# mpkuse/cerebro

Measured on AMD Instinct MI355X. Metric: loop-queries/sec (ticks of 3 descriptors vs 4096-D x 1M DB), higher is better.
Workload: dtype f64

## Files before the change

cerebro_amd/csrc/chip_api.hip:

```cpp
#include "chip_internal.h"
#include <cmath>
#include <cstdlib>
#include <cstring>
#include <memory>
#include <new>

using namespace chip;

extern "C" {

const char *chip_strerror(int status)
{
    switch (status) {
        case CHIP_OK: return "ok";
        case CHIP_ERR_INVALID_ARG: return "invalid argument";
        case CHIP_ERR_NO_DEVICE: return "no usable HIP device";
        case CHIP_ERR_HIP: return "HIP runtime error (see chip_last_hip_error)";
        case CHIP_ERR_OOM: return "out of device memory";
        case CHIP_ERR_NOT_F32: return "descriptor value not exactly representable as float32";
        case CHIP_ERR_NONFINITE: return "NaN/Inf in descriptor";
        case CHIP_ERR_RANGE: return "index / length out of range";
        case CHIP_ERR_UNSUPPORTED: return "unsupported configuration";
        case CHIP_ERR_TOO_FEW_POINTS: return "fewer than 20 correspondences";
        case CHIP_ERR_BUSY: return "async slot busy or empty";
// ... 157 lines not shown
    c->scan_overlap_bytes = (double)env_int("CHIP_SCAN_OVERLAP_GIB", 8) * 1024 * 1024 * 1024;
    c->scan_reserve = env_int("CHIP_SCAN_RESERVE", c->nranks > 1 ? 4 : 0);
    c->max_grid = 512;
    c->scan_streams = env_int("CHIP_SCAN_STREAMS", c->nranks > 1 ? 2 : 4);
    c->tick_fused = env_int("CHIP_TICK_FUSED", 1) != 0;
}

static int create_impl(chip_ctx *c, int64_t capacity_hint, int elem)
{
    hipDeviceProp_t prop;
    CHIP_HIP(c, hipGetDeviceProperties(&prop, c->device));
    c->n_cus = prop.multiProcessorCount;
    std::strncpy(c->arch, prop.gcnArchName, sizeof(c->arch) - 1);
    if (std::strncmp(c->arch, "gfx950", 6) != 0 && !std::getenv("CHIP_ALLOW_ANY_ARCH")) return CHIP_ERR_NO_DEVICE;

    c->segs.reserve(kMaxSegs);

    CHIP_HIP(c, hipStreamCreateWithFlags(&c->s_query, hipStreamNonBlocking));
    CHIP_HIP(c, hipStreamCreateWithFlags(&c->s_append, hipStreamNonBlocking));
    CHIP_HIP(c, hipStreamCreateWithFlags(&c->s_pnp, hipStreamNonBlocking));
    int rc = c->seg_table_dev.alloc(c, kMaxSegs);
    if (rc == CHIP_OK) rc = configure_storage(c, elem);
    if (rc != CHIP_OK) return rc;
    c->stage_bytes = 64ull << 20;
    if (c->stage_bytes < (size_t)c->D * 8 * 64) c->stage_bytes = (size_t)c->D * 8 * 64;
    rc = c->stage_dev.alloc(c, c->stage_bytes);
    if (rc == CHIP_OK) rc = c->flags_dev.alloc(c, 1);
    if (rc == CHIP_OK) rc = c->flags_host.alloc(c, 1);
    if (rc == CHIP_OK) rc = c->norm2_dev.alloc(c, 1);
    if (rc == CHIP_OK) rc = c->norm2_host.alloc(c, 1);
    if (rc != CHIP_OK) return rc;
    CHIP_HIP(c, hipMemset(c->norm2_dev, 0, sizeof(unsigned long long)));
    *c->norm2_host.host() = 0;

    scan_read_knobs(c);
    CHIP_HIP(c, hipStreamCreateWithFlags(&c->s_scan, hipStreamNonBlocking));
    {
        const int ns = c->scan_streams;
        if (ns >= 2) CHIP_HIP(c, hipStreamCreateWithFlags(&c->s_scan2, hipStreamNonBlocking));
        for (int i = 0; i < 2; i++)
            if (ns >= 3 + i) CHIP_HIP(c, hipStreamCreateWithFlags(&c->s_scan_x[i], hipStreamNonBlocking));
    }
    for (int i = 0; i < Ctx::kRing; i++) {
        constexpr size_t kListsPerGroup = 3 * kPrefilterTicks > CHIP_MAX_NQ ? 3 * kPrefilterTicks : CHIP_MAX_NQ;
        static_assert(kPrefilterTicks >= kMultiMaxTicks, "the list buffers are sized for the deepest pass");
        rc = c->partial_dev[i].alloc(c, ((size_t)c->max_grid + 1) * kListsPerGroup * CHIP_MAX_TOPK);
        if (rc != CHIP_OK) return rc;
        CHIP_HIP(c, hipEventCreateWithFlags(&c->ev_scan[i], hipEventDisableTiming));
        CHIP_HIP(c, hipEventCreateWithFlags(&c->ev_merged[i], hipEventDisableTiming));
    }
    rc = c->tickets_dev.alloc(c, Ctx::kRing);
    if (rc != CHIP_OK) return rc;
    CHIP_HIP(c, hipMemset(c->tickets_dev, 0, Ctx::kRing * sizeof(int32_t)));
    c->coalesce_max = env_int("CHIP_TICK_COALESCE", kPrefilterTicks);
    if (c->coalesce_max < 2) c->coalesce_max = 0;
    if (c->coalesce_max > kPrefilterTicks) c->coalesce_max = kPrefilterTicks;
    c->tick_poll = env_int("CHIP_TICK_POLL", 1) != 0;
    resident_read_knobs(c);
    rc = c->seq_all.alloc(c, CHIP_MAX_INFLIGHT);
    if (rc != CHIP_OK) return rc;
    std::memset(c->seq_all.host(), 0, sizeof(unsigned long long) * CHIP_MAX_INFLIGHT);
    rc = c->cert_all.alloc(c, CHIP_MAX_INFLIGHT * 4);
    if (rc != CHIP_OK) return rc;
    std::memset(c->cert_all.host(), 0, sizeof(uint32_t) * CHIP_MAX_INFLIGHT * 4);
    rc = c->topk.alloc(c, (size_t)CHIP_MAX_NQ * CHIP_MAX_TOPK);
    if (rc != CHIP_OK) return rc;
    for (Slot &s : c->slots) {
        CHIP_HIP(c, hipEventCreateWithFlags(&s.done, hipEventDisableTiming));
        rc = s.rec.alloc(c, 1);
        if (rc != CHIP_OK) return rc;
        s.seq_host = c->seq_all.host() + (&s - c->slots);
        s.seq_dev = c->seq_all.dev() + (&s - c->slots);
        s.cert_host = c->cert_all.host() + 4 * (&s - c->slots);
        s.cert_dev = c->cert_all.dev() + 4 * (&s - c->slots);
    }
    if (env_int("CHIP_SCAN_STAMPS", 0)) {
        rc = c->stamps_dev.alloc(c, (size_t)c->max_grid * 16 * 4 + 64);
        if (rc != CHIP_OK) return rc;
        CHIP_HIP(c, hipMemset(c->stamps_dev, 0, ((size_t)c->max_grid * 16 * 4 + 64) * sizeof(unsigned long long)));
    }
    rc = pnp_create(c);
    if (rc != CHIP_OK) return rc;
    c->cap_hint = capacity_hint;
    if (capacity_hint > 0) {
        std::lock_guard<std::mutex> lk(c->append_mu);
        rc = ensure_capacity(c, local_count(c, capacity_hint));
        if (rc != CHIP_OK) return rc;
    }
    return CHIP_OK;
}

int ctx_create(chip_ctx **out, int32_t D, int64_t capacity_hint, int32_t device, int32_t shard_rank, int32_t shard_count, uint32_t flags)
{
    if (!out) return CHIP_ERR_INVALID_ARG;
    *out = nullptr;
    if (D <= 0 || shard_count < 1 || shard_rank < 0 || shard_rank >= shard_count || capacity_hint < 0) return CHIP_ERR_INVALID_ARG;
    const uint32_t store = flags & kCreateStoreMask;
    if (store == kCreateStoreMask) return CHIP_ERR_INVALID_ARG;
    if (D % 4 != 0 || (size_t)D * 4 * CHIP_MAX_NQ > 160 * 1024) return CHIP_ERR_UNSUPPORTED;
    if (store == CHIP_CREATE_STORE_F64 && (size_t)D * 8 * 2 > 160 * 1024) return CHIP_ERR_UNSUPPORTED;
    int ndev = 0;
    if (hipGetDeviceCount(&ndev) != hipSuccess || ndev <= 0) return CHIP_ERR_NO_DEVICE;
    if (device < 0 || device >= ndev) return CHIP_ERR_NO_DEVICE;
    if (hipSetDevice(device) != hipSuccess) return CHIP_ERR_NO_DEVICE;
    chip_ctx *c = new (std::nothrow) chip_ctx();
    if (!c) return CHIP_ERR_OOM;
// ... 220 lines not shown
    const int rc = enqueue_scan_merge(c, rq, &done);
    if (rc != CHIP_OK) return rc;
    if (done.done_ev) s.wait_ev = done.done_ev;
    else { CHIP_HIP(c, hipEventRecord(s.done, done.merge_stream)); s.wait_ev = s.done; }
    s.pass_no = c->pass_no;
    s.state = c->tick_poll && done.fused ? SlotState::Poll : SlotState::Event;
    return CHIP_OK;
}

int coalesce_decide(int n_parked, int t_max, bool scan_running)
{
    if (t_max < 2) return kCoalesceLaunch;
    if (!scan_running) return n_parked > 0 ? kCoalesceParkFlush : kCoalesceLaunch;
    return n_parked + 1 >= t_max ? kCoalesceParkFlush : kCoalescePark;
}

static int coalesce_ticks_max(const Ctx *c, int64_t k, bool sync_tick)
{
    if (c->coalesce_max < 2 || sync_tick || c->nranks != 1 || c->xchg || c->parent || c->group || !c->own_query_stream) return 0;
    if ((double)k * c->D * c->elem <= c->scan_overlap_bytes) return 0;
    int fit = scan_multi_max_ticks(c);
    if (c->coalesce_max >= kPrefilterTicks && scan_prefilter_usable(c)) fit = kPrefilterTicks;
    const int t = fit < c->coalesce_max ? fit : c->coalesce_max;
    return t >= 2 ? t : 0;
}

static int coalesce_submit(Ctx *c, int T)
{
    const int b = (int)(c->n_enqueued++ % Ctx::kRing);
    const int K = CHIP_DEFAULT_TOPK;
    const bool prefilter = T == kPrefilterTicks;
    static_assert(kPrefilterTicks > kMultiMaxTicks, "a pass of kPrefilterTicks ticks is the prefilter's");
    PassArgs a{};
    scan_args_db(c, &a);
    a.K = K;
    a.partial = c->partial_dev[b];
    for (int t = 0; t < T; t++) {
        a.k[t] = c->parked[t].k;
        if (a.k[t] > a.n_rows) a.n_rows = a.k[t];
        for (int i = 0; i < 3; i++) a.q[3 * t + i] = c->parked[t].q[i];
    }
    const int grid = scan_multi_grid(c);
    double E = 0.0;
    if (prefilter) {
        std::lock_guard<std::mutex> lk(c->mu);
        E = prefilter_error_bound(c->D, c->row_norm_max);
    }
    if (hipEventQuery(c->ev_merged[b]) != hipSuccess) CHIP_HIP(c, hipStreamWaitEvent(c->s_scan, c->ev_merged[b], 0));
    hipEvent_t e1 = nullptr;
    int rc = c->prof_on ? prof_begin(c, c->s_scan, (double)a.n_rows * c->D * c->elem, &e1) : CHIP_OK;
    if (rc == CHIP_OK) rc = prefilter ? launch_scan_prefilter(c, c->s_scan, a, grid) : launch_scan_multi(c, c->s_scan, a, T, grid);
    if (rc != CHIP_OK) return rc;
    if (e1) CHIP_HIP(c, hipEventRecord(e1, c->s_scan));
    CHIP_HIP(c, hipEventRecord(c->ev_scan[b], c->s_scan));
    c->pass_ev = c->ev_scan[b];
    c->pass_no++;
    CHIP_HIP(c, hipStreamWaitEvent(c->s_query, c->ev_scan[b], 0));
    chip_topk_entry *exact = c->partial_dev[b] + (size_t)kPrefilterTicks * grid * 3 * K;
    if (prefilter) {
        RescoreArgs ra{};
        ra.seg_table = a.seg_table; ra.seg_shift = a.seg_shift; ra.seg_mask = a.seg_mask; ra.D = a.D; ra.K = K;
        ra.in = c->partial_dev[b]; ra.n_lists = grid; ra.wpb = 8;
        ra.E = E;
        ra.out = exact;
        for (int t = 0; t < T; t++) {
            const Ctx::ParkedTick &pt = c->parked[t];
            Slot &s = *pt.slot;
            ra.k[t] = pt.k;
            for (int i = 0; i < 3; i++) { ra.q[3 * t + i] = s.pf_q[i] = pt.q[i]; s.cert_host[i] = 0; }
            ra.cert[t] = s.cert_dev;
            s.prefilter = true; s.pf_k = pt.k; s.pf_p = pt.p;
        }
        rc = launch_rescore(c, c->s_query, ra);
        if (rc != CHIP_OK) return rc;
    }
    for (int t = 0; t < T; t++) {
        const Ctx::ParkedTick &pt = c->parked[t];
        if (prefilter) rc = launch_merge(c, c->s_query, merge_args(exact + (size_t)t * 3 * K, 1, K, nullptr, pt.slot->rec.dev(), pt.l, &pt.p), 3);
        else rc = launch_merge(c, c->s_query, merge_args(c->partial_dev[b] + (size_t)t * grid * 3 * K, grid, K, nullptr, pt.slot->rec.dev(), pt.l, &pt.p), 3);
        if (rc != CHIP_OK) return rc;
        CHIP_HIP(c, hipEventRecord(pt.slot->done, c->s_query));
        pt.slot->wait_ev = pt.slot->done;
        pt.slot->state = SlotState::Event;
        pt.slot->pass_no = c->pass_no;
    }
    CHIP_HIP(c, hipEventRecord(c->ev_merged[b], c->s_query));
    c->coalesce_passes++;
    c->coalesce_ticks += T;
    if (prefilter) { c->prefilter_passes++; c->prefilter_ticks += T; }
    return CHIP_OK;
}

int coalesce_flush(Ctx *c)
{
    const int T = c->n_parked;
    if (T == 0) return CHIP_OK;
    c->n_parked = 0;
    const Ctx::ParkedTick &p0 = c->parked[0];
    int rc;
    if (T == kPrefilterTicks && !scan_prefilter_usable(c)) {
        const Ctx::ParkedTick &pl = c->parked[T - 1];
        rc = coalesce_submit(c, T - 1);
        if (rc == CHIP_OK) rc = tick_submit(c, pl.k, pl.l, &pl.p, pl.q, false, *pl.slot);
    } else {
        rc = T == 1 ? tick_submit(c, p0.k, p0.l, &p0.p, p0.q, false, *p0.slot) : coalesce_submit(c, T);
    }
    for (int t = 0; t < T && rc != CHIP_OK; t++) {
        c->parked[t].slot->state = SlotState::Failed;
        c->parked[t].slot->err = rc;
    }
    return rc;
}

static int tick_enqueue_slot(Ctx *c, int64_t l, const chip_dot_params *p, bool sync_tick, Slot &s)
{
    int32_t status = 0;
    int64_t k = 0;
    const int64_t n_pub = published_rows(c);
    int rc = tick_begin(s, c->xchg ? INT64_MAX : n_pub, &c->last_l, l, p, &status, &k);
    if (rc != CHIP_OK || status != CHIP_TICK_SCANNED) return rc;
    if (c->xchg) {
        rc = xchg_tick_enqueue(c, l, k, p, sync_tick, s, l > n_pub);
        if (rc != CHIP_OK) return rc;
    } else {
        const int64_t rows[3] = {l - 1, l - 2, l - 3};
        const void *q[3];
        RingGuard rg(c);
        rc = query_row_ptrs(c, rows, 3, l, q);
        if (rc != CHIP_OK) return rc;
        if (resident_eligible(c, k)) {
            (void)coalesce_flush(c);
            rc = resident_tick_enqueue(c, k, l, p, s);
            if (rc == CHIP_OK) { c->last_l = l; return CHIP_OK; }
            if (rc != CHIP_ERR_UNSUPPORTED && rc != kResidentPaused) return rc;
        }
        const int t_max = coalesce_ticks_max(c, k, sync_tick);
        const int act = t_max < 2 ? kCoalesceLaunch
                                  : coalesce_decide(c->n_parked, t_max, c->coalesce_force || (c->pass_ev && hipEventQuery(c->pass_ev) == hipErrorNotReady));
        if (act == kCoalesceLaunch) {
// ... 809 lines not shown
```

cerebro_amd/csrc/chip_internal.h:

```cpp
#pragma once
#include <hip/hip_runtime.h>
#include <cstdint>
#include <mutex>
#include <condition_variable>
#include <vector>
#include "../../include/cerebro_hip.h"

namespace chip {

constexpr int kWave = 64;
constexpr int kMaxSegs = 4096;
constexpr int64_t kSegBytesTarget = 512ll << 20;

struct ScanArgs {
    const void *const *seg_table;
    int32_t seg_shift;
    int64_t seg_mask;
    int64_t n_rows;
    int32_t D;
    int32_t K;
    const void *q[CHIP_MAX_NQ];
    int64_t idx_mul, idx_add;
    chip_topk_entry *partial;
    int32_t q64 = 0;
    int32_t rows_form = 0;
    int32_t plain_loads = 0;
    int32_t dyn_claim = 0;
    unsigned long long *stamps = nullptr;
    chip_tick_result *fused_result = nullptr;
    int32_t *fused_ticket = nullptr;
    unsigned long long *fused_seq = nullptr;
    unsigned long long fused_seq_val = 0;
    int64_t tick_l = 0;
    int32_t locality = 0;
    double thresh = 0.0;
};

struct ResidentCmd {
    uint32_t head;
    int32_t locality;
    int64_t n_rows;
    int64_t tick_l;
    double thresh;
    uint64_t result;
    uint64_t seq_ptr;
    uint64_t seq_val;
    uint32_t dyn_claim;
    uint32_t tail;
};
static_assert(sizeof(ResidentCmd) == 64, "one cache line, one PCIe read");
constexpr uint32_t kResidentLeave = 0xffffffffu;

struct ResidentArgs {
    ScanArgs base;
    const uint32_t *cmd_host;
    uint32_t *cmd_dev;
    unsigned long long *exit_host;
    unsigned long long instance;
    unsigned long long lease_ticks;
    uint32_t done;
    uint32_t direct;
};

constexpr int kMultiMaxTicks = 3;
constexpr int kPrefilterTicks = 4;
constexpr int kRescoreCap = 32;
struct PassArgs {
    const void *const *seg_table;
    int32_t seg_shift;
    int64_t seg_mask;
    int64_t n_rows;
    int32_t D;
    int32_t K;
    int64_t k[kPrefilterTicks];
    const void *q[3 * kPrefilterTicks];
    chip_topk_entry *partial;
};
struct RescoreArgs {
    const void *const *seg_table;
    int32_t seg_shift;
    int64_t seg_mask;
    int32_t D;
    int32_t K;
    const chip_topk_entry *in;
    int32_t n_lists;
    int32_t wpb;
    int64_t k[kPrefilterTicks];
    const void *q[3 * kPrefilterTicks];
    double E;
    chip_topk_entry *out;
    uint32_t *cert[kPrefilterTicks];
};

struct MergeArgs {
    const chip_topk_entry *in;
    int32_t n_lists;
    int32_t K;
    chip_topk_entry *out;
    chip_tick_result *result;
    int64_t l;
    int32_t locality;
    double thresh;
};

struct Ctx;

template <class T> class DevBuf {
public:
    DevBuf() = default;
    DevBuf(const DevBuf &) = delete;
    DevBuf &operator=(const DevBuf &) = delete;
    ~DevBuf() { release(); }
    int alloc(Ctx *c, size_t n);
    int reserve(Ctx *c, size_t n);
    void release() { if (p_) (void)hipFree(p_); p_ = nullptr; cap_ = 0; }
    T *get() const { return p_; }
    operator T *() const { return p_; }
    size_t capacity() const { return cap_; }
private:
    T *p_ = nullptr;
    size_t cap_ = 0;
};
template <class T> class PinnedBuf {
public:
    PinnedBuf() = default;
    PinnedBuf(const PinnedBuf &) = delete;
    PinnedBuf &operator=(const PinnedBuf &) = delete;
    ~PinnedBuf() { release(); }
    int alloc(Ctx *c, size_t n);
    int reserve(Ctx *c, size_t n);
    void release() { if (h_) (void)hipHostFree(h_); h_ = d_ = nullptr; cap_ = 0; }
    T *host() const { return h_; }
    T *dev() const { return d_; }
    size_t capacity() const { return cap_; }
private:
    T *h_ = nullptr, *d_ = nullptr;
    size_t cap_ = 0;
};

int launch_resident(Ctx *c, hipStream_t s, const ResidentArgs &ra, int grid);
int launch_scan(Ctx *c, hipStream_t s, const ScanArgs &a, int nq, int grid);
int launch_merge(Ctx *c, hipStream_t s, const MergeArgs &a, int nq);
int scan_multi_max_ticks(const Ctx *c);
int scan_multi_plan(int D, int elem, int n_ticks, int K, int grid, chip_debug_scan_launch *f);
int scan_multi_grid(const Ctx *c);
int launch_scan_multi(Ctx *c, hipStream_t s, const PassArgs &a, int n_ticks, int grid);
int scan_prefilter_plan(int D, int elem, int K, int grid, chip_debug_scan_launch *f);
bool scan_prefilter_usable(const Ctx *c);
double prefilter_error_bound(int D, double row_norm_max);
int launch_scan_prefilter(Ctx *c, hipStream_t s, const PassArgs &a, int grid);
int launch_rescore(Ctx *c, hipStream_t s, const RescoreArgs &a);
int scan_grid_for(const Ctx *c, int64_t n_rows, int nq, bool q64);
bool scan_q64(const Ctx *c, int nq, bool long_scan);
int scan_rows_form(const Ctx *c, int64_t n_rows, int nq, int grid, bool q64, bool sync_tick = false);
int scan_select(const Ctx *c, const ScanArgs &a, int nq, int grid, chip_debug_scan_launch *f);
int scan_forms_built();
int launch_scores(Ctx *c, hipStream_t s, const ScanArgs &a, double *out_dev);
int launch_store_rows(Ctx *c, hipStream_t s, const void *src, int src_elem, int64_t n, int64_t first_global, uint32_t *flags_dev, bool write_ring,
                      int64_t row_stride = 1);
int launch_synth(Ctx *c, hipStream_t s, int64_t first_global, int64_t n, uint64_t seed,
                 const int64_t *plant_dst_dev, const int64_t *plant_src_dev, const int32_t *plant_kind_dev, int64_t n_plant, int unit);

enum class SlotState : uint8_t {
    Free,
    Immediate,
    Parked,
    Event,
    Poll,
    Resident,
    Failed,
};

struct Slot {
    hipEvent_t done = nullptr;
    hipEvent_t wait_ev = nullptr;
    PinnedBuf<chip_tick_result> rec;
    SlotState state = SlotState::Free;
    int64_t prev_last_l = 0;
    int64_t tick_l = 0;
    unsigned long long *seq_host = nullptr, *seq_dev = nullptr;
    unsigned long long seq_want = 0;
    uint64_t pass_no = 0;
    int32_t err = 0;
    bool prefilter = false;
    uint32_t *cert_host = nullptr, *cert_dev = nullptr;
    int64_t pf_k = 0;
    chip_dot_params pf_p{};
    const void *pf_q[3] = {};
    int64_t *last_l_ptr = nullptr;
};

struct Resident {
    bool enabled = false;
    double max_bytes = 512.0 * 1024 * 1024;
    int32_t lease_ms = 250;
// ... 29 lines not shown
struct MatchState;
struct OrbState;
struct Exchange;
struct Group;

struct Ctx {
    int32_t D = 0;
    int32_t device = 0;
    int32_t rank = 0, nranks = 1;
    int32_t n_cus = 0;
    char arch[32] = {0};

    int32_t elem = 4;
    bool store_auto = true;

    int32_t seg_shift = 0;
    int64_t seg_rows = 0;
    std::vector<void *> segs;
    DevBuf<void *> seg_table_dev;
    DevBuf<char> ring_dev;
    int64_t rows_global = 0;
    int64_t rows_local = 0;
    int64_t lossy_rows = 0;
    mutable std::mutex mu;
    std::mutex append_mu;
    mutable std::mutex query_mu;
    std::mutex ring_mu;
    int64_t rows_pending = 0;
    hipEvent_t last_scan_ev[2] = {};
    std::mutex pnp_mu;
    std::mutex icp_mu;

    hipStream_t s_query = nullptr, s_append = nullptr, s_pnp = nullptr;
    bool own_query_stream = true;

    DevBuf<char> stage_dev;
    size_t stage_bytes = 0;
    DevBuf<uint32_t> flags_dev;
    PinnedBuf<uint32_t> flags_host;
    DevBuf<unsigned long long> norm2_dev;
    PinnedBuf<unsigned long long> norm2_host;
    double row_norm_max = 0.0;

    static constexpr int kRing = 64;
    hipStream_t s_scan = nullptr;
    hipStream_t s_scan2 = nullptr;
    hipStream_t s_scan_x[2] = {};
    uint64_t n_same_stream = 0;
    DevBuf<chip_topk_entry> partial_dev[kRing];
    int32_t partial_lists[kRing] = {};
    hipEvent_t ev_scan[kRing] = {};
    hipEvent_t ev_merged[kRing] = {};
    DevBuf<int32_t> tickets_dev;
    PinnedBuf<unsigned long long> seq_all;
    unsigned long long tick_seq = 0;
    bool tick_poll = true;
    bool tick_fused = true;
    Resident res;
    uint64_t n_enqueued = 0;
    int32_t max_grid = 0;
    PinnedBuf<chip_topk_entry> topk;

    DevBuf<char> qvec_dev;
    DevBuf<double> scores_dev;
    DevBuf<unsigned long long> stamps_dev;

    std::vector<char> qconv;
    int64_t cap_hint = 0;
    int32_t group_transport = 0;
    mutable int last_comm = 0;
    int32_t comm_init_abandoned = 0;
    Exchange *xchg = nullptr;
    Group *group = nullptr;
    Ctx *parent = nullptr;
    Slot slots[CHIP_MAX_INFLIGHT];
    int64_t last_l = 0;

    struct ParkedTick { Slot *slot; int64_t k, l; chip_dot_params p; const void *q[3]; };
    int32_t coalesce_max = 4;
    bool coalesce_force = false;
    ParkedTick parked[kPrefilterTicks];
    int32_t n_parked = 0;
    hipEvent_t pass_ev = nullptr;
    uint64_t pass_no = 0;
    int64_t coalesce_passes = 0, coalesce_ticks = 0;
    int64_t prefilter_passes = 0, prefilter_ticks = 0, prefilter_uncertified = 0;
    PinnedBuf<uint32_t> cert_all;
    chip_debug_scan_launch last_scan{};

    int32_t scan_block = 0;
    int32_t scan_blocks_per_cu = 2;
    int32_t scan_reserve = 0;
    int32_t scan_variant = 0;
    int32_t scan_streams = 4;
    bool tick_same_stream = true;
    int32_t scan_claim = -1;
    int32_t scan_rows = 0;
    double scan_plain_bytes = 768.0 * 1024 * 1024;
    double scan_sync_plain_bytes = 4096.0 * 1024 * 1024;
    double scan_half_bytes = 192.0 * 1024 * 1024;
    int32_t scan_short_bpc = 1;
    double scan_overlap_bytes = 8.0 * 1024 * 1024 * 1024;

    bool prof_on = false;
    std::vector<hipEvent_t> prof_ev;
    size_t prof_used = 0;
// ... 197 lines not shown
```

cerebro_amd/csrc/kernels.hip:

```cpp
#include "chip_internal.h"
#include "topk_merge.h"
#include <cmath>
#include <type_traits>

namespace chip {

typedef float f32x4 __attribute__((ext_vector_type(4)));
typedef double f64x2 __attribute__((ext_vector_type(2)));

template <typename T> struct Vec16;
template <> struct Vec16<float> { typedef f32x4 type; static constexpr int N = 4; };
template <> struct Vec16<double> { typedef f64x2 type; static constexpr int N = 2; };

template <typename V>
__device__ __forceinline__ const __attribute__((address_space(1))) V *as_global(const V *p)
{
    return (const __attribute__((address_space(1))) V *)p;
}

template <typename V>
__device__ __forceinline__ V stream_load(const V *p)
{
    return __builtin_nontemporal_load(as_global(p));
}
// ... 611 lines not shown
        static_for<U>([&](auto uc) CHIP_INLINE_LAMBDA {
            constexpr int u = uc;
            slot_wait<L - R>();
            static_for<NS>([&](auto qc) CHIP_INLINE_LAMBDA {
                constexpr int q = qc, i = u * NS + q;
                if constexpr (i + 2 < SS) w[i + 2] = *reinterpret_cast<const f32x4 *>(qv + ((i + 2) % NS) * D + ((i + 2) / NS) * 256);
                const f32x2 wl = __builtin_shufflevector(w[i], w[i], 0, 1), wh = __builtin_shufflevector(w[i], w[i], 2, 3);
                static_for<R>([&](auto rr) CHIP_INLINE_LAMBDA { prefilter_fma<pass_row_slot(u, rr)>(acc[rr][q], wl); });
                static_for<R>([&](auto rr) CHIP_INLINE_LAMBDA { prefilter_fma<pass_row_slot(u, rr) + 2>(acc[rr][q], wh); });
                __builtin_amdgcn_sched_barrier(0);
            });
            static_for<NG>([&](auto gc) CHIP_INLINE_LAMBDA {
                constexpr int g = gc, QR = pass_query_slot(NG, u, g);
                slot_wait<L - R - 1 - g>();
                static_for<R>([&](auto rr) CHIP_INLINE_LAMBDA { prefilter_fma_slot<pass_row_slot(u, rr), QR>(acc[rr][NS + g]); });
                static_for<R>([&](auto rr) CHIP_INLINE_LAMBDA { prefilter_fma_slot<pass_row_slot(u, rr) + 2, QR + 2>(acc[rr][NS + g]); });
            });
            slots_issue_kib<u, NG>(voff, row, qg);
        });
    }
};

template <int NG>
__global__ __launch_bounds__(kMultiBlock) __attribute__((amdgpu_num_vgpr(pass_vgpr_base(kPrefilterMaxNG) / 2))) void db_scan_prefilter(PassArgs a)
{
    static_assert(NG <= kPrefilterMaxNG, "the compiler's share is sized for kPrefilterMaxNG query slots per KiB");
    shared_pass<PassF32<NG>>(a);
}

__device__ __forceinline__ void block_best(double &bs, int64_t &bi, double *red_s, int64_t *red_i, int lane, int wave)
{
#pragma unroll
    for (int m = 32; m >= 1; m >>= 1) {
        const double os = __shfl_xor(bs, m, 64);
        const int64_t oi = __shfl_xor(bi, m, 64);
        if (key_gt(os, oi, bs, bi)) { bs = os; bi = oi; }
    }
    __syncthreads();
    if (lane == 0) { red_s[wave] = bs; red_i[wave] = bi; }
    __syncthreads();
    bs = red_s[0]; bi = red_i[0];
#pragma unroll
    for (int w = 1; w < 8; w++)
        if (key_gt(red_s[w], red_i[w], bs, bi)) { bs = red_s[w]; bi = red_i[w]; }
}

__global__ __launch_bounds__(512) void tick_rescore(RescoreArgs a)
{
    constexpr int MAXH = 512 * CHIP_MAX_TOPK / 512;
    __shared__ double red_s[8];
    __shared__ int64_t red_i[8];
    __shared__ chip_topk_entry cand[kRescoreCap];
    __shared__ int n_cand;
    const int tid = threadIdx.x, lane = tid & 63;
    const int wave = __builtin_amdgcn_readfirstlane(tid >> 6);
    const int tick = blockIdx.x / 3, q = blockIdx.x % 3;
    const int K = a.K, n = a.n_lists * K;
    const chip_topk_entry *in = a.in + (int64_t)tick * a.n_lists * 3 * K;
    const int64_t k = a.k[tick];
    if (tid == 0) n_cand = 0;
    double es[MAXH];
    int64_t ei[MAXH];
#pragma unroll
    for (int h = 0; h < MAXH; h++) {
        const int c = tid + 512 * h;
        es[h] = -INFINITY; ei[h] = -1;
        if (c < n) { const chip_topk_entry t = in[((int64_t)(c / K) * 3 + q) * K + (c % K)]; es[h] = t.score; ei[h] = t.idx; }
    }
    double ms = -INFINITY;
    int64_t mi = -1;
    const int64_t tw = (int64_t)a.n_lists * a.wpb;
#pragma unroll
    for (int h = 0; h < MAXH; h++) {
        const int c = tid + 512 * h;
        if (c % K != K - 1 || ei[h] < 0) continue;
        int64_t part = k % tw - (int64_t)(c / K) * a.wpb;
        part = part < 0 ? 0 : part > a.wpb ? a.wpb : part;
        if ((k / tw) * a.wpb + part > K && es[h] > ms) { ms = es[h]; mi = 0; }
    }
    block_best(ms, mi, red_s, red_i, lane, wave);
    double gs = INFINITY;
    int64_t gi = INT64_MAX;
    for (int j = 0; j < K; j++) {
        double bs = -INFINITY;
        int64_t bi = -1;
#pragma unroll
        for (int h = 0; h < MAXH; h++)
            if (key_gt(gs, gi, es[h], ei[h]) && key_gt(es[h], ei[h], bs, bi)) { bs = es[h]; bi = ei[h]; }
        block_best(bs, bi, red_s, red_i, lane, wave);
        gs = bs; gi = bi;
    }
    double thr = gs - 2.0 * a.E;
    thr -= fabs(thr) * 0x1p-51;
    const bool ok = mi < 0 || ms < thr;
#pragma unroll
    for (int h = 0; h < MAXH; h++)
        if (ei[h] >= 0 && es[h] >= thr) {
            const int at = atomicAdd(&n_cand, 1);
            if (at < kRescoreCap) { chip_topk_entry t; t.score = es[h]; t.idx = ei[h]; cand[at] = t; }
        }
    __syncthreads();
    const int nc = n_cand < kRescoreCap ? n_cand : kRescoreCap;
    const float *qrow = static_cast<const float *>(a.q[3 * tick + q]);
    for (int j = wave; j < nc; j += 8) {
        const int64_t r = cand[j].idx;
        const float *row[1] = {static_cast<const float *>(a.seg_table[r >> a.seg_shift]) + (r & a.seg_mask) * (int64_t)a.D};
        double acc[1][1];
        rows_dot<float, 1, 4, true, 1, 1>(row, qrow, a.D, lane, acc);
        const double s = butterfly_sum(acc[0][0]);
        if (lane == 0) cand[j].score = s;
    }
    __syncthreads();
    if (wave == 0) {
        static_assert(kRescoreCap <= 64, "one lane per candidate");
        chip_topk_entry *out = a.out + (int64_t)(3 * tick + q) * K;
        chip_topk_entry me;
        me.score = -INFINITY; me.idx = -1;
        if (lane < nc) me = cand[lane];
        int rank = 0;
        for (int j = 0; j < nc; j++) {
            const chip_topk_entry o = cand[j];
            rank += key_gt(o.score, o.idx, me.score, me.idx) ? 1 : 0;
        }
        if (lane < nc && rank < K) out[rank] = me;
        if (lane >= nc && lane < K) out[lane] = me;
        if (lane == 0) a.cert[tick][q] = ok && n_cand <= kRescoreCap ? 1u : 2u;
    }
}

template <int NQ, int NG, bool FULL>
__global__ __launch_bounds__(1024) void db_scan_topk_wide(ScanArgs a)
{
    static_assert(NG >= 1 && NG < NQ, "at least one query staged, at least one read in place");
    extern __shared__ __attribute__((aligned(16))) char smem[];
    double *qs = reinterpret_cast<double *>(smem);
    constexpr int NL = NQ - NG, U = 4, CH = 128;
    const int D = a.D, K = a.K;
    const int tid = threadIdx.x, lane = tid & 63;
    const int wave = __builtin_amdgcn_readfirstlane(tid >> 6);
    const int wpb = blockDim.x >> 6;
    stage_queries<double, NL>(a, qs, tid, blockDim.x);
    __syncthreads();
    const double *qg[NG];
#pragma unroll
    for (int g = 0; g < NG; g++) qg[g] = static_cast<const double *>(a.q[NL + g]);

    double my_s[NQ], thr_s[NQ];
    int64_t my_i[NQ], thr_i[NQ];
#pragma unroll
    for (int q = 0; q < NQ; q++) { my_s[q] = -INFINITY; my_i[q] = -1; thr_s[q] = -INFINITY; thr_i[q] = -1; }
    const int e0 = lane * 2;
    const int64_t tw = (int64_t)gridDim.x * wpb;
    for (int64_t r = (int64_t)blockIdx.x * wpb + wave; r < a.n_rows; r += tw) {
        const double *row = row_base<double>(a, r);
        double acc[NQ];
#pragma unroll
        for (int q = 0; q < NQ; q++) acc[q] = 0.0;
        for (int base = 0; base < D; base += CH * U) {
            f64x2 v[U];
#pragma unroll
            for (int u = 0; u < U; u++) {
                const int e = base + u * CH + e0;
                if (FULL || e < D) v[u] = __builtin_nontemporal_load(as_global(reinterpret_cast<const f64x2 *>(row + e)));
            }
#pragma unroll
            for (int u = 0; u < U; u++) {
                const int e = base + u * CH + e0;
                if (FULL || e < D) {
#pragma unroll
                    for (int q = 0; q < NQ; q++) {
                        const f64x2 w = q < NL ? *reinterpret_cast<const f64x2 *>(qs + q * D + e)
                                               : *as_global(reinterpret_cast<const f64x2 *>(qg[q < NL ? 0 : q - NL] + e));
                        acc[q] = __builtin_fma(w[0], v[u][0], acc[q]);
                        acc[q] = __builtin_fma(w[1], v[u][1], acc[q]);
                    }
                }
            }
        }
#pragma unroll
        for (int q = 0; q < NQ; q++) acc[q] = butterfly_sum(acc[q]);
// ... 884 lines not shown
#else
    int block, bpc;
    scan_shape(c, 3, false, &block, &bpc);
    const size_t lds = scan_lds_bytes(c, 3, 1, block, false, true);
    if (lds + 64 > 160 * 1024 || grid > 512) return CHIP_ERR_UNSUPPORTED;
    return c->elem == 8 ? launch_resident_T<double>(c, s, ra, grid, lds, block) : launch_resident_T<float>(c, s, ra, grid, lds, block);
#endif
}

template <typename T, bool FULL>
__global__ __launch_bounds__(512) void db_scan_scores(ScanArgs a, double *out)
{
    extern __shared__ __attribute__((aligned(16))) char smem[];
    T *qs = reinterpret_cast<T *>(smem);
    const int tid = threadIdx.x, lane = tid & 63;
    const int wave = __builtin_amdgcn_readfirstlane(tid >> 6);
    const int wpb = blockDim.x >> 6;
    stage_queries<T, 1>(a, qs, tid, blockDim.x);
    __syncthreads();
    const int64_t tw = (int64_t)gridDim.x * wpb;
    for (int64_t r = (int64_t)blockIdx.x * wpb + wave; r < a.n_rows; r += tw) {
        const T *row[1] = {row_base<T>(a, r)};
        double acc[1][1];
        rows_dot<T, 1, 4, FULL, FULL ? 6 : 1, 1>(row, qs, a.D, lane, acc);
        const double s = butterfly_sum(acc[0][0]);
        if (lane == 0) out[r] = s;
    }
}

int launch_scores(Ctx *c, hipStream_t s, const ScanArgs &a, double *out_dev)
{
    const size_t lds = (size_t)c->D * c->elem;
    int64_t grid = (a.n_rows + 7) / 8;
    if (grid > (int64_t)c->n_cus * 4) grid = (int64_t)c->n_cus * 4;
    if (grid < 1) grid = 1;
    const int chunk = 64 * (16 / c->elem) * 4;
    const bool full = a.D % chunk == 0;
    if (c->elem == 8) {
        if (lds > 65536) {
            CHIP_HIP(c, hipFuncSetAttribute(reinterpret_cast<const void *>(db_scan_scores<double, true>), hipFuncAttributeMaxDynamicSharedMemorySize, (int)lds));
            CHIP_HIP(c, hipFuncSetAttribute(reinterpret_cast<const void *>(db_scan_scores<double, false>), hipFuncAttributeMaxDynamicSharedMemorySize, (int)lds));
        }
        if (full) hipLaunchKernelGGL((db_scan_scores<double, true>), dim3((int)grid), dim3(512), lds, s, a, out_dev);
        else hipLaunchKernelGGL((db_scan_scores<double, false>), dim3((int)grid), dim3(512), lds, s, a, out_dev);
    } else {
        if (full) hipLaunchKernelGGL((db_scan_scores<float, true>), dim3((int)grid), dim3(512), lds, s, a, out_dev);
        else hipLaunchKernelGGL((db_scan_scores<float, false>), dim3((int)grid), dim3(512), lds, s, a, out_dev);
    }
    CHIP_HIP(c, hipGetLastError());
    return CHIP_OK;
}

template <int NQ>
__global__ __launch_bounds__(512) void topk_merge(MergeArgs a)
{
    __shared__ __attribute__((aligned(16))) char smem[kMergeSmem];
    merge_sorted_lists<NQ>(a.in, a.n_lists, NQ, 0, a.K, a.out, a.result, a.l, a.locality, a.thresh, smem);
}

int launch_merge(Ctx *c, hipStream_t s, const MergeArgs &a, int nq)
{
    if (a.n_lists > 512) return CHIP_ERR_UNSUPPORTED;
    switch (nq) {
        case 1: hipLaunchKernelGGL(topk_merge<1>, dim3(1), dim3(512), 0, s, a); break;
        case 2: hipLaunchKernelGGL(topk_merge<2>, dim3(1), dim3(512), 0, s, a); break;
        case 3: hipLaunchKernelGGL(topk_merge<3>, dim3(1), dim3(512), 0, s, a); break;
        case 4: hipLaunchKernelGGL(topk_merge<4>, dim3(1), dim3(512), 0, s, a); break;
        default: return CHIP_ERR_UNSUPPORTED;
    }
    CHIP_HIP(c, hipGetLastError());
    return CHIP_OK;
}

struct StoreArgs {
    void *const *seg_table;
    int32_t seg_shift;
    int64_t seg_mask;
    void *ring;
    int32_t D;
    int32_t rank, nranks;
    int64_t first_global;
    int64_t row_stride;
    int64_t n;
    int64_t ring_from;
    uint32_t *flags;
};

template <typename T>
__device__ __forceinline__ void store_row4(const StoreArgs &a, int64_t g, int e, const T (&v)[4])
{
    typedef typename Vec16<T>::type V;
    constexpr int N = Vec16<T>::N;
    V pk[4 / N];
#pragma unroll
    for (int c = 0; c < 4; c++) pk[c / N][c % N] = v[c];
    if (a.nranks == 1 || (g % a.nranks) == a.rank) {
        const int64_t loc = a.nranks == 1 ? g : g / a.nranks;
        T *dst = static_cast<T *>(a.seg_table[loc >> a.seg_shift]) + (loc & a.seg_mask) * (int64_t)a.D + e;
#pragma unroll
        for (int h = 0; h < 4 / N; h++) reinterpret_cast<V *>(dst)[h] = pk[h];
    }
    if (a.ring && g >= a.ring_from) {
        T *dst = static_cast<T *>(a.ring) + (g % CHIP_RING_ROWS) * (int64_t)a.D + e;
#pragma unroll
        for (int h = 0; h < 4 / N; h++) reinterpret_cast<V *>(dst)[h] = pk[h];
    }
}

template <typename S, typename T>
__global__ __launch_bounds__(256) void convert_rows(StoreArgs a, const S *__restrict__ src)
{
    const int64_t per_row = a.D / 4;
    const int64_t total = a.n * per_row;
    uint32_t bad = 0;
    for (int64_t i = (int64_t)blockIdx.x * blockDim.x + threadIdx.x; i < total; i += (int64_t)gridDim.x * blockDim.x) {
        const int64_t r = i / per_row;
        const int e = (int)(i - r * per_row) * 4;
        S x[4];
        if constexpr (sizeof(S) == 8) {
            const f64x2 lo = *reinterpret_cast<const f64x2 *>(src + r * a.D + e);
            const f64x2 hi = *reinterpret_cast<const f64x2 *>(src + r * a.D + e + 2);
            x[0] = lo.x; x[1] = lo.y; x[2] = hi.x; x[3] = hi.y;
// ... 212 lines not shown
```

cerebro_amd/csrc/topk_merge.h:

```cpp
#pragma once
#include "chip_internal.h"
#include <cmath>

namespace chip {

__device__ __forceinline__ bool key_gt(double s, int64_t i, double s2, int64_t i2)
{
    return s > s2 || (s == s2 && i > i2);
}

constexpr int kMergeSmem = 28 * 1024;
constexpr int64_t kFailedShardIdx = -2;
constexpr int kSurvCap = CHIP_MAX_TOPK * CHIP_MAX_TOPK;

__device__ __forceinline__ double readlane_f64(double v, int j)
{
    const long long b = __double_as_longlong(v);
    const int lo = __builtin_amdgcn_readlane((int)(b & 0xffffffffll), j);
    const int hi = __builtin_amdgcn_readlane((int)(b >> 32), j);
    return __longlong_as_double(((long long)hi << 32) | (unsigned int)lo);
}
__device__ __forceinline__ int64_t readlane_i64(int64_t v, int j)
{
    const int lo = __builtin_amdgcn_readlane((int)(v & 0xffffffffll), j);
    const int hi = __builtin_amdgcn_readlane((int)(v >> 32), j);
    return ((int64_t)hi << 32) | (unsigned int)lo;
}

__device__ __forceinline__ unsigned long long okey(double s)
{
    const unsigned long long b0 = (unsigned long long)__double_as_longlong(s);
    const unsigned long long b = b0 == 0x8000000000000000ull ? 0ull : b0;
    return (b >> 63) ? ~b : (b | 0x8000000000000000ull);
}

__device__ __forceinline__ int wave_rank(double s, int64_t i, bool valid)
{
    const unsigned kh = (unsigned)(okey(s) >> 32);
    int rank = 0, eq = 0;
#pragma unroll 16
    for (int j = 0; j < 64; j++) {
        const unsigned o = (unsigned)__builtin_amdgcn_readlane((int)kh, j);
        rank += o > kh ? 1 : 0;
        eq += o == kh ? 1 : 0;
    }
    if (__ballot(valid && eq > 1) == 0ull) return rank;
    rank = 0;
#pragma unroll 8
    for (int j = 0; j < 64; j++) rank += key_gt(readlane_f64(s, j), readlane_i64(i, j), s, i) ? 1 : 0;
    return rank;
}

__device__ __forceinline__ void wave_rank2(const double s[2], const int64_t i[2], int &r0, int &r1)
{
    const unsigned k0 = (unsigned)(okey(s[0]) >> 32), k1 = (unsigned)(okey(s[1]) >> 32);
    int e0 = 0, e1 = 0;
    r0 = r1 = 0;
#pragma unroll 16
    for (int j = 0; j < 64; j++) {
        const unsigned a = (unsigned)__builtin_amdgcn_readlane((int)k0, j), b = (unsigned)__builtin_amdgcn_readlane((int)k1, j);
        r0 += (a > k0 ? 1 : 0) + (b > k0 ? 1 : 0);
        e0 += (a == k0 ? 1 : 0) + (b == k0 ? 1 : 0);
        r1 += (a > k1 ? 1 : 0) + (b > k1 ? 1 : 0);
        e1 += (a == k1 ? 1 : 0) + (b == k1 ? 1 : 0);
    }
    if (__ballot((i[0] >= 0 && e0 > 1) || (i[1] >= 0 && e1 > 1)) == 0ull) return;
    r0 = r1 = 0;
#pragma unroll 8
    for (int j = 0; j < 64; j++) {
        const double a0 = readlane_f64(s[0], j), a1 = readlane_f64(s[1], j);
        const int64_t b0 = readlane_i64(i[0], j), b1 = readlane_i64(i[1], j);
        r0 += (key_gt(a0, b0, s[0], i[0]) ? 1 : 0) + (key_gt(a1, b1, s[0], i[0]) ? 1 : 0);
        r1 += (key_gt(a0, b0, s[1], i[1]) ? 1 : 0) + (key_gt(a1, b1, s[1], i[1]) ? 1 : 0);
    }
}

template <int NQ>
__device__ __forceinline__ void merge_sorted_lists(const chip_topk_entry *in, int n_lists, int list_stride, int q_off, int K, chip_topk_entry *out,
                                                   chip_tick_result *result, int64_t l, int locality, double thresh, char *smem)
{
    chip_topk_entry *candA = reinterpret_cast<chip_topk_entry *>(smem);
    chip_topk_entry *surv = candA + CHIP_MAX_NQ * 8 * CHIP_MAX_TOPK;
    chip_topk_entry *T1s = surv + CHIP_MAX_NQ * kSurvCap;
    chip_topk_entry *tops = T1s + CHIP_MAX_NQ;
    int *cnt = reinterpret_cast<int *>(tops + CHIP_MAX_NQ);
    int *failed = cnt + CHIP_MAX_NQ;
    const int t = threadIdx.x;
    const int lane = t & 63, w = t >> 6, nw = blockDim.x >> 6;

    double hs[NQ];
    int64_t hi[NQ];
#pragma unroll
    for (int q = 0; q < NQ; q++) {
        if (t < n_lists) { const chip_topk_entry x = in[((int64_t)t * list_stride + q_off + q) * K]; hs[q] = x.score; hi[q] = x.idx; }
        else { hs[q] = -INFINITY; hi[q] = -1; }
    }
    if (t < NQ) cnt[t] = 0;
    if (t == NQ) *failed = 0;
#pragma unroll
    for (int q = 0; q < NQ; q++) {
        const bool valid = hi[q] >= 0;
        const int rank = wave_rank(hs[q], hi[q], valid);
        const int nvalid = __popcll(__ballot(valid));
        chip_topk_entry *dst = candA + (q * 8 + w) * CHIP_MAX_TOPK;
        if (valid && rank < K) { dst[rank].score = hs[q]; dst[rank].idx = hi[q]; }
        if (lane < K && lane >= nvalid) { dst[lane].score = -INFINITY; dst[lane].idx = -1; }
    }
    __syncthreads();
    if (t < n_lists && hi[0] == kFailedShardIdx) *failed = 1;
    if (w < NQ) {
        const int q = w;
        double cs[2];
        int64_t ci[2];
#pragma unroll
        for (int h = 0; h < 2; h++) {
            const int c = lane + 64 * h;
            if (c < nw * K) { const chip_topk_entry x = candA[(q * 8 + c / K) * CHIP_MAX_TOPK + (c % K)]; cs[h] = x.score; ci[h] = x.idx; }
            else { cs[h] = -INFINITY; ci[h] = -1; }
        }
        int r0, r1;
        wave_rank2(cs, ci, r0, r1);
        const int nv = __popcll(__ballot(ci[0] >= 0)) + __popcll(__ballot(ci[1] >= 0));
        if (nv >= K) {
            if (ci[0] >= 0 && r0 == K - 1) { T1s[q].score = cs[0]; T1s[q].idx = ci[0]; }
            if (ci[1] >= 0 && r1 == K - 1) { T1s[q].score = cs[1]; T1s[q].idx = ci[1]; }
        } else if (lane == 0) { T1s[q].score = -INFINITY; T1s[q].idx = -1; }
    }
    __syncthreads();
#pragma unroll
    for (int q = 0; q < NQ; q++) {
        const double ts = T1s[q].score;
        const int64_t ti = T1s[q].idx;
        if (t < n_lists && hi[q] >= 0 && !key_gt(ts, ti, hs[q], hi[q])) {
            double es[CHIP_MAX_TOPK];
            int64_t ei[CHIP_MAX_TOPK];
            es[0] = hs[q]; ei[0] = hi[q];
#pragma unroll
            for (int j = 1; j < CHIP_MAX_TOPK; j++) {
                if (j < K) { const chip_topk_entry x = in[((int64_t)t * list_stride + q_off + q) * K + j]; es[j] = x.score; ei[j] = x.idx; }
                else { es[j] = -INFINITY; ei[j] = -1; }
            }
            int c = 1;
#pragma unroll
            for (int j = 1; j < CHIP_MAX_TOPK; j++)
                if (c == j && ei[j] >= 0 && !key_gt(ts, ti, es[j], ei[j])) c = j + 1;
            const int base = atomicAdd(&cnt[q], c);
#pragma unroll
            for (int j = 0; j < CHIP_MAX_TOPK; j++)
                if (j < c && base + j < kSurvCap) { surv[q * kSurvCap + base + j].score = es[j]; surv[q * kSurvCap + base + j].idx = ei[j]; }
        }
    }
    __syncthreads();
    if (w < NQ) {
        const int q = w;
        int n = cnt[q];
        if (n > kSurvCap) n = kSurvCap;
        double cs[4];
        int64_t ci[4];
        int rk[4];
#pragma unroll
        for (int h = 0; h < 4; h++) {
            const int c = lane + 64 * h;
            if (c < n) { cs[h] = surv[q * kSurvCap + c].score; ci[h] = surv[q * kSurvCap + c].idx; }
            else { cs[h] = -INFINITY; ci[h] = -1; }
            rk[h] = 0;
        }
        for (int j = 0; j < n; j++) {
            const chip_topk_entry x = surv[q * kSurvCap + j];
#pragma unroll
            for (int h = 0; h < 4; h++) rk[h] += key_gt(x.score, x.idx, cs[h], ci[h]) ? 1 : 0;
        }
#pragma unroll
        for (int h = 0; h < 4; h++) {
            if (ci[h] >= 0 && rk[h] < K) {
                if (out) { out[q * K + rk[h]].score = cs[h]; out[q * K + rk[h]].idx = ci[h]; }
                if (rk[h] == 0) { tops[q].score = cs[h]; tops[q].idx = ci[h]; }
            }
        }
        if (lane < K && lane >= n) {
            if (out) { out[q * K + lane].score = -INFINITY; out[q * K + lane].idx = -1; }
            if (lane == 0) { tops[q].score = -INFINITY; tops[q].idx = -1; }
        }
    }
    __syncthreads();
    if (out != nullptr && t == 0 && *failed) out[0].idx = kFailedShardIdx;
    if (result != nullptr && t == 0) {
        chip_tick_result res;
        res.status = *failed ? CHIP_TICK_FAILED : CHIP_TICK_SCANNED;
        res.found = 0;
        res.idx_curr = -1;
        res.idx_prev = -1;
        res.score = 0.0;
        for (int q = 0; q < 3; q++) {
            res.argmax[q] = q < NQ ? tops[q].idx : -1;
            res.maxv[q] = q < NQ ? tops[q].score : -INFINITY;
        }
        if (NQ >= 3 && res.argmax[0] >= 0 && res.argmax[1] >= 0 && res.argmax[2] >= 0) {
            int64_t d1 = res.argmax[0] - res.argmax[1];
            int64_t d2 = res.argmax[0] - res.argmax[2];
            if (d1 < 0) d1 = -d1;
            if (d2 < 0) d2 = -d2;
            if (d1 < locality && d2 < locality && res.maxv[0] > thresh) {
                res.found = 1;
                res.idx_curr = l - 1;
                res.idx_prev = res.argmax[0];
                res.score = res.maxv[0];
            }
        }
        *result = res;
    }
}


}
```

Baseline: 1216.

## Fuse per-tick merges into rescore via last-block ticket and batch merge launch

```diff
diff --git a/cerebro_amd/csrc/chip_api.hip b/cerebro_amd/csrc/chip_api.hip
--- a/cerebro_amd/csrc/chip_api.hip
+++ b/cerebro_amd/csrc/chip_api.hip
@@ -233,6 +233,9 @@
     rc = c->tickets_dev.alloc(c, Ctx::kRing);
     if (rc != CHIP_OK) return rc;
     CHIP_HIP(c, hipMemset(c->tickets_dev, 0, Ctx::kRing * sizeof(int32_t)));
+    rc = c->pass_tickets_dev.alloc(c, (size_t)Ctx::kRing * kPrefilterTicks);
+    if (rc != CHIP_OK) return rc;
+    CHIP_HIP(c, hipMemset(c->pass_tickets_dev, 0, (size_t)Ctx::kRing * kPrefilterTicks * sizeof(int32_t)));
     c->coalesce_max = env_int("CHIP_TICK_COALESCE", kPrefilterTicks);
     if (c->coalesce_max < 2) c->coalesce_max = 0;
     if (c->coalesce_max > kPrefilterTicks) c->coalesce_max = kPrefilterTicks;
@@ -559,10 +562,6 @@
     if (rc == CHIP_OK) rc = prefilter ? launch_scan_prefilter(c, c->s_scan, a, grid) : launch_scan_multi(c, c->s_scan, a, T, grid);
     if (rc != CHIP_OK) return rc;
     if (e1) CHIP_HIP(c, hipEventRecord(e1, c->s_scan));
-    CHIP_HIP(c, hipEventRecord(c->ev_scan[b], c->s_scan));
-    c->pass_ev = c->ev_scan[b];
-    c->pass_no++;
-    CHIP_HIP(c, hipStreamWaitEvent(c->s_query, c->ev_scan[b], 0));
     chip_topk_entry *exact = c->partial_dev[b] + (size_t)kPrefilterTicks * grid * 3 * K;
     if (prefilter) {
         RescoreArgs ra{};
@@ -570,28 +569,35 @@
         ra.in = c->partial_dev[b]; ra.n_lists = grid; ra.wpb = 8;
         ra.E = E;
         ra.out = exact;
+        ra.tickets = c->pass_tickets_dev + (size_t)b * kPrefilterTicks;
         for (int t = 0; t < T; t++) {
             const Ctx::ParkedTick &pt = c->parked[t];
             Slot &s = *pt.slot;
             ra.k[t] = pt.k;
             for (int i = 0; i < 3; i++) { ra.q[3 * t + i] = s.pf_q[i] = pt.q[i]; s.cert_host[i] = 0; }
             ra.cert[t] = s.cert_dev;
+            ra.fin[t] = merge_args(exact + (size_t)t * 3 * K, 1, K, nullptr, s.rec.dev(), pt.l, &pt.p);
             s.prefilter = true; s.pf_k = pt.k; s.pf_p = pt.p;
         }
-        rc = launch_rescore(c, c->s_query, ra);
-        if (rc != CHIP_OK) return rc;
-    }
+        rc = launch_rescore(c, c->s_scan, ra);
+    } else {
+        MergeLaunchArgs m{};
+        for (int t = 0; t < T; t++) {
+            const Ctx::ParkedTick &pt = c->parked[t];
+            m.t[t] = merge_args(c->partial_dev[b] + (size_t)t * grid * 3 * K, grid, K, nullptr, pt.slot->rec.dev(), pt.l, &pt.p);
+        }
+        rc = launch_merge_ticks(c, c->s_scan, m, T);
+    }
+    if (rc != CHIP_OK) return rc;
+    CHIP_HIP(c, hipEventRecord(c->ev_merged[b], c->s_scan));
+    c->pass_ev = c->ev_merged[b];
+    c->pass_no++;
     for (int t = 0; t < T; t++) {
-        const Ctx::ParkedTick &pt = c->parked[t];
-        if (prefilter) rc = launch_merge(c, c->s_query, merge_args(exact + (size_t)t * 3 * K, 1, K, nullptr, pt.slot->rec.dev(), pt.l, &pt.p), 3);
-        else rc = launch_merge(c, c->s_query, merge_args(c->partial_dev[b] + (size_t)t * grid * 3 * K, grid, K, nullptr, pt.slot->rec.dev(), pt.l, &pt.p), 3);
-        if (rc != CHIP_OK) return rc;
-        CHIP_HIP(c, hipEventRecord(pt.slot->done, c->s_query));
-        pt.slot->wait_ev = pt.slot->done;
-        pt.slot->state = SlotState::Event;
-        pt.slot->pass_no = c->pass_no;
-    }
-    CHIP_HIP(c, hipEventRecord(c->ev_merged[b], c->s_query));
+        Slot &s = *c->parked[t].slot;
+        s.wait_ev = c->ev_merged[b];
+        s.state = SlotState::Event;
+        s.pass_no = c->pass_no;
+    }
     c->coalesce_passes++;
     c->coalesce_ticks += T;
     if (prefilter) { c->prefilter_passes++; c->prefilter_ticks += T; }
diff --git a/cerebro_amd/csrc/chip_internal.h b/cerebro_amd/csrc/chip_internal.h
--- a/cerebro_amd/csrc/chip_internal.h
+++ b/cerebro_amd/csrc/chip_internal.h
@@ -76,6 +76,20 @@
     const void *q[3 * kPrefilterTicks];
     chip_topk_entry *partial;
 };
+struct MergeArgs {
+    const chip_topk_entry *in;
+    int32_t n_lists;
+    int32_t K;
+    chip_topk_entry *out;
+    chip_tick_result *result;
+    int64_t l;
+    int32_t locality;
+    double thresh;
+};
+struct MergeLaunchArgs {
+    MergeArgs t[kPrefilterTicks];
+};
+
 struct RescoreArgs {
     const void *const *seg_table;
     int32_t seg_shift;
@@ -90,17 +104,8 @@
     double E;
     chip_topk_entry *out;
     uint32_t *cert[kPrefilterTicks];
-};
-
-struct MergeArgs {
-    const chip_topk_entry *in;
-    int32_t n_lists;
-    int32_t K;
-    chip_topk_entry *out;
-    chip_tick_result *result;
-    int64_t l;
-    int32_t locality;
-    double thresh;
+    MergeArgs fin[kPrefilterTicks];
+    int32_t *tickets;
 };
 
 struct Ctx;
@@ -141,6 +146,7 @@
 int launch_resident(Ctx *c, hipStream_t s, const ResidentArgs &ra, int grid);
 int launch_scan(Ctx *c, hipStream_t s, const ScanArgs &a, int nq, int grid);
 int launch_merge(Ctx *c, hipStream_t s, const MergeArgs &a, int nq);
+int launch_merge_ticks(Ctx *c, hipStream_t s, const MergeLaunchArgs &m, int n_ticks);
 int scan_multi_max_ticks(const Ctx *c);
 int scan_multi_plan(int D, int elem, int n_ticks, int K, int grid, chip_debug_scan_launch *f);
 int scan_multi_grid(const Ctx *c);
@@ -276,6 +282,7 @@
     hipEvent_t ev_scan[kRing] = {};
     hipEvent_t ev_merged[kRing] = {};
     DevBuf<int32_t> tickets_dev;
+    DevBuf<int32_t> pass_tickets_dev;
     PinnedBuf<unsigned long long> seq_all;
     unsigned long long tick_seq = 0;
     bool tick_poll = true;
diff --git a/cerebro_amd/csrc/kernels.hip b/cerebro_amd/csrc/kernels.hip
--- a/cerebro_amd/csrc/kernels.hip
+++ b/cerebro_amd/csrc/kernels.hip
@@ -687,6 +687,7 @@
     __shared__ int64_t red_i[8];
     __shared__ chip_topk_entry cand[kRescoreCap];
     __shared__ int n_cand;
+    __shared__ __attribute__((aligned(16))) char fin_smem[merge_smem_bytes<1, CHIP_MAX_TOPK>()];
     const int tid = threadIdx.x, lane = tid & 63;
     const int wave = __builtin_amdgcn_readfirstlane(tid >> 6);
     const int tick = blockIdx.x / 3, q = blockIdx.x % 3;
@@ -761,6 +762,21 @@
         if (lane >= nc && lane < K) out[lane] = me;
         if (lane == 0) a.cert[tick][q] = ok && n_cand <= kRescoreCap ? 1u : 2u;
     }
+    asm volatile("s_waitcnt vmcnt(0)" ::: "memory");
+    __syncthreads();
+    if (tid == 0) {
+        __builtin_amdgcn_fence(__ATOMIC_RELEASE, "agent");
+        asm volatile("s_waitcnt vmcnt(0)" ::: "memory");
+        n_cand = __hip_atomic_fetch_add(a.tickets + tick, 1, __ATOMIC_RELAXED, __HIP_MEMORY_SCOPE_AGENT) == 2 ? 1 : 0;
+        if (n_cand) {
+            __builtin_amdgcn_fence(__ATOMIC_ACQUIRE, "agent");
+            asm volatile("s_waitcnt vmcnt(0)" ::: "memory");
+        }
+    }
+    __syncthreads();
+    if (!n_cand) return;
+    merge_lists<3, 1, CHIP_MAX_TOPK>(a.fin[tick], fin_smem);
+    if (tid == 0) __hip_atomic_store(a.tickets + tick, 0, __ATOMIC_RELAXED, __HIP_MEMORY_SCOPE_AGENT);
 }
 
 template <int NQ, int NG, bool FULL>
@@ -1751,22 +1767,34 @@
 }
 
 template <int NQ>
-__global__ __launch_bounds__(512) void topk_merge(MergeArgs a)
+__global__ __launch_bounds__(512) void topk_merge(MergeLaunchArgs a)
 {
     __shared__ __attribute__((aligned(16))) char smem[kMergeSmem];
-    merge_sorted_lists<NQ>(a.in, a.n_lists, NQ, 0, a.K, a.out, a.result, a.l, a.locality, a.thresh, smem);
+    merge_lists<NQ>(a.t[blockIdx.x], smem);
 }
 
 int launch_merge(Ctx *c, hipStream_t s, const MergeArgs &a, int nq)
 {
     if (a.n_lists > 512) return CHIP_ERR_UNSUPPORTED;
+    MergeLaunchArgs m{};
+    m.t[0] = a;
     switch (nq) {
-        case 1: hipLaunchKernelGGL(topk_merge<1>, dim3(1), dim3(512), 0, s, a); break;
-        case 2: hipLaunchKernelGGL(topk_merge<2>, dim3(1), dim3(512), 0, s, a); break;
-        case 3: hipLaunchKernelGGL(topk_merge<3>, dim3(1), dim3(512), 0, s, a); break;
-        case 4: hipLaunchKernelGGL(topk_merge<4>, dim3(1), dim3(512), 0, s, a); break;
+        case 1: hipLaunchKernelGGL(topk_merge<1>, dim3(1), dim3(512), 0, s, m); break;
+        case 2: hipLaunchKernelGGL(topk_merge<2>, dim3(1), dim3(512), 0, s, m); break;
+        case 3: hipLaunchKernelGGL(topk_merge<3>, dim3(1), dim3(512), 0, s, m); break;
+        case 4: hipLaunchKernelGGL(topk_merge<4>, dim3(1), dim3(512), 0, s, m); break;
         default: return CHIP_ERR_UNSUPPORTED;
     }
+    CHIP_HIP(c, hipGetLastError());
+    return CHIP_OK;
+}
+
+int launch_merge_ticks(Ctx *c, hipStream_t s, const MergeLaunchArgs &m, int n_ticks)
+{
+    if (n_ticks < 1 || n_ticks > kPrefilterTicks) return CHIP_ERR_UNSUPPORTED;
+    for (int t = 0; t < n_ticks; t++)
+        if (m.t[t].n_lists > 512) return CHIP_ERR_UNSUPPORTED;
+    hipLaunchKernelGGL(topk_merge<3>, dim3(n_ticks), dim3(512), 0, s, m);
     CHIP_HIP(c, hipGetLastError());
     return CHIP_OK;
 }
diff --git a/cerebro_amd/csrc/topk_merge.h b/cerebro_amd/csrc/topk_merge.h
--- a/cerebro_amd/csrc/topk_merge.h
+++ b/cerebro_amd/csrc/topk_merge.h
@@ -75,13 +75,18 @@
     }
 }
 
-template <int NQ>
+template <int NW, int SURV>
+constexpr int merge_smem_bytes() { return (CHIP_MAX_NQ * NW * CHIP_MAX_TOPK + CHIP_MAX_NQ * SURV + 2 * CHIP_MAX_NQ) * (int)sizeof(chip_topk_entry) + (CHIP_MAX_NQ + 1) * (int)sizeof(int); }
+static_assert(merge_smem_bytes<8, kSurvCap>() <= kMergeSmem, "the general merge fits kMergeSmem");
+
+template <int NQ, int NW = 8, int SURV = kSurvCap>
 __device__ __forceinline__ void merge_sorted_lists(const chip_topk_entry *in, int n_lists, int list_stride, int q_off, int K, chip_topk_entry *out,
                                                    chip_tick_result *result, int64_t l, int locality, double thresh, char *smem)
 {
+    static_assert(NW >= 1 && NW <= 8 && SURV >= CHIP_MAX_TOPK && SURV <= kSurvCap, "list heads of at most 8 waves, survivors of at least one list");
     chip_topk_entry *candA = reinterpret_cast<chip_topk_entry *>(smem);
-    chip_topk_entry *surv = candA + CHIP_MAX_NQ * 8 * CHIP_MAX_TOPK;
-    chip_topk_entry *T1s = surv + CHIP_MAX_NQ * kSurvCap;
+    chip_topk_entry *surv = candA + CHIP_MAX_NQ * NW * CHIP_MAX_TOPK;
+    chip_topk_entry *T1s = surv + CHIP_MAX_NQ * SURV;
     chip_topk_entry *tops = T1s + CHIP_MAX_NQ;
     int *cnt = reinterpret_cast<int *>(tops + CHIP_MAX_NQ);
     int *failed = cnt + CHIP_MAX_NQ;
@@ -102,9 +107,11 @@
         const bool valid = hi[q] >= 0;
         const int rank = wave_rank(hs[q], hi[q], valid);
         const int nvalid = __popcll(__ballot(valid));
-        chip_topk_entry *dst = candA + (q * 8 + w) * CHIP_MAX_TOPK;
-        if (valid && rank < K) { dst[rank].score = hs[q]; dst[rank].idx = hi[q]; }
-        if (lane < K && lane >= nvalid) { dst[lane].score = -INFINITY; dst[lane].idx = -1; }
+        if (NW == 8 || w < NW) {
+            chip_topk_entry *dst = candA + (q * NW + w) * CHIP_MAX_TOPK;
+            if (valid && rank < K) { dst[rank].score = hs[q]; dst[rank].idx = hi[q]; }
+            if (lane < K && lane >= nvalid) { dst[lane].score = -INFINITY; dst[lane].idx = -1; }
+        }
     }
     __syncthreads();
     if (t < n_lists && hi[0] == kFailedShardIdx) *failed = 1;
@@ -115,7 +122,7 @@
 #pragma unroll
         for (int h = 0; h < 2; h++) {
             const int c = lane + 64 * h;
-            if (c < nw * K) { const chip_topk_entry x = candA[(q * 8 + c / K) * CHIP_MAX_TOPK + (c % K)]; cs[h] = x.score; ci[h] = x.idx; }
+            if (c < (NW == 8 || nw < NW ? nw : NW) * K) { const chip_topk_entry x = candA[(q * NW + c / K) * CHIP_MAX_TOPK + (c % K)]; cs[h] = x.score; ci[h] = x.idx; }
             else { cs[h] = -INFINITY; ci[h] = -1; }
         }
         int r0, r1;
@@ -147,31 +154,32 @@
             const int base = atomicAdd(&cnt[q], c);
 #pragma unroll
             for (int j = 0; j < CHIP_MAX_TOPK; j++)
-                if (j < c && base + j < kSurvCap) { surv[q * kSurvCap + base + j].score = es[j]; surv[q * kSurvCap + base + j].idx = ei[j]; }
+                if (j < c && base + j < SURV) { surv[q * SURV + base + j].score = es[j]; surv[q * SURV + base + j].idx = ei[j]; }
         }
     }
     __syncthreads();
     if (w < NQ) {
         const int q = w;
         int n = cnt[q];
-        if (n > kSurvCap) n = kSurvCap;
-        double cs[4];
-        int64_t ci[4];
-        int rk[4];
-#pragma unroll
-        for (int h = 0; h < 4; h++) {
+        if (n > SURV) n = SURV;
+        constexpr int H = (SURV + 63) / 64;
+        double cs[H];
+        int64_t ci[H];
+        int rk[H];
+#pragma unroll
+        for (int h = 0; h < H; h++) {
             const int c = lane + 64 * h;
-            if (c < n) { cs[h] = surv[q * kSurvCap + c].score; ci[h] = surv[q * kSurvCap + c].idx; }
+            if (c < n) { cs[h] = surv[q * SURV + c].score; ci[h] = surv[q * SURV + c].idx; }
             else { cs[h] = -INFINITY; ci[h] = -1; }
             rk[h] = 0;
         }
         for (int j = 0; j < n; j++) {
-            const chip_topk_entry x = surv[q * kSurvCap + j];
-#pragma unroll
-            for (int h = 0; h < 4; h++) rk[h] += key_gt(x.score, x.idx, cs[h], ci[h]) ? 1 : 0;
-        }
-#pragma unroll
-        for (int h = 0; h < 4; h++) {
+            const chip_topk_entry x = surv[q * SURV + j];
+#pragma unroll
+            for (int h = 0; h < H; h++) rk[h] += key_gt(x.score, x.idx, cs[h], ci[h]) ? 1 : 0;
+        }
+#pragma unroll
+        for (int h = 0; h < H; h++) {
             if (ci[h] >= 0 && rk[h] < K) {
                 if (out) { out[q * K + rk[h]].score = cs[h]; out[q * K + rk[h]].idx = ci[h]; }
                 if (rk[h] == 0) { tops[q].score = cs[h]; tops[q].idx = ci[h]; }
@@ -211,5 +219,10 @@
     }
 }
 
-
-}
+template <int NQ, int NW = 8, int SURV = kSurvCap>
+__device__ __forceinline__ void merge_lists(const MergeArgs &a, char *smem)
+{
+    merge_sorted_lists<NQ, NW, SURV>(a.in, a.n_lists, NQ, 0, a.K, a.out, a.result, a.l, a.locality, a.thresh, smem);
+}
+
+}
```

After: 1219, median of 3. No clear change (+0.2%).
